# idiap/ilqr_planner

Hardware: AMD Instinct MI355X
Metric: iLQR iterations/sec (7-DoF, T=200, batch 4096) + final-cost rel-err vs Eigen ref (higher is better)
Workload: dtype f64; 1 GPU; C3: PosOrn nb_deriv=1 7-DoF Panda chain, T=200, batch 4096/GPU x 1 GPU = 4096, solver=al, 20 iterations/solve, line search on, early stop off; global_batch=4096, horizon=200, parallelism=instances sharded x1, exchange=none

## Files before the change

### ilqr_planner_amd/capi.py

```python
from __future__ import annotations

import collections
import ctypes as C
import os

import numpy as np

_HERE = os.path.dirname(os.path.abspath(__file__))
LIB_PATH = os.path.join(_HERE, "libilqr_hip.so")

MAX_SEG, MAX_KP, MAX_NX, MAX_NU, MAX_NF, MAX_NQ = 24, 8, 15, 8, 15, 13
SYS_POS_ORN, SYS_POS_ORN_TIME, SYS_JOINT, SYS_JOINT_TIME = 0, 1, 2, 3
STATUS_OK, STATUS_NONFINITE, STATUS_ALPHA_FLOOR = 0, 1, 2
LQT_MAX_NX, LQT_MAX_NU = 16, 8
CL_STATS = 5
KP_ERR, KP_STATS, CL_OUTCOME = 5, 12, 4
KP_ERR_POS, KP_ERR_ORN, KP_ERR_VEL, KP_ERR_ANGVEL, KP_ERR_TIME = range(5)
PROF_ROLLOUT, PROF_BACKWARD, PROF_FORWARD, PROF_OTHER, PROF_APPLY = 0, 1, 2, 3, 4

EXPORTS = [
    "ilqr_dims_of", "ilqr_desc_defaults", "ilqr_ctx_create", "ilqr_ctx_destroy", "ilqr_last_error", "ilqr_ctx_set_stream",
    "ilqr_ctx_synchronize", "ilqr_version", "ilqr_problem_create", "ilqr_problem_destroy", "ilqr_problem_set_init_state",
    "ilqr_problem_set_keypoint_targets", "ilqr_problem_set_controls", "ilqr_problem_set_constraints",
    "ilqr_problem_set_init_state_dev", "ilqr_problem_set_keypoint_targets_dev", "ilqr_problem_set_controls_dev",
    "ilqr_solve_recursive", "ilqr_solve_al", "ilqr_solve_batch_cp", "ilqr_solve_batch", "ilqr_problem_get_X", "ilqr_problem_get_fX",
    "ilqr_problem_get_U", "ilqr_problem_get_K", "ilqr_problem_get_d", "ilqr_problem_get_cost", "ilqr_problem_get_alpha",
    "ilqr_problem_get_iters", "ilqr_problem_get_status", "ilqr_problem_get_lambda", "ilqr_problem_get_trace",
    "ilqr_problem_get_X_dev", "ilqr_problem_get_U_dev", "ilqr_problem_get_cost_dev", "ilqr_fk_batch",
    "ilqr_profile_enable", "ilqr_profile_reset", "ilqr_profile_get", "ilqr_chain_from_urdf", "ilqr_urdf_last_error",
    "ilqr_problem_reset_multipliers", "ilqr_problem_warm_start", "ilqr_problem_track", "ilqr_problem_track_dev",
    "ilqr_problem_closed_loop", "ilqr_problem_closed_loop_dev", "ilqr_problem_closed_loop_noise", "ilqr_problem_closed_loop_noise_dev",
    "ilqr_problem_closed_loop_report", "ilqr_problem_closed_loop_report_dev",
    "ilqr_ctx_set_split", "ilqr_ctx_set_crosscheck",
    "ilqr_lqt_create", "ilqr_lqt_destroy", "ilqr_lqt_set_targets", "ilqr_lqt_set_targets_dev", "ilqr_lqt_solve_dp", "ilqr_lqt_solve_lin_al",
    "ilqr_lqt_command", "ilqr_lqt_command_dev", "ilqr_lqt_get_U", "ilqr_lqt_get_U_dev", "ilqr_lqt_get_X", "ilqr_lqt_get_X_dev", "ilqr_lqt_get_P",
    "ilqr_lqt_get_d",
]


class ProblemDesc(C.Structure):

    _fields_ = [
        ("kind", C.c_int),
        ("nb_deriv", C.c_int),
        ("dof", C.c_int),
        ("horizon", C.c_int),
        ("dt", C.c_double),
        ("R_diag", C.c_double * MAX_NU),
        ("limits_set", C.c_int),
        ("penalty", C.c_double),
        ("state_max", C.c_double * (MAX_NX + 1)),
        ("state_min", C.c_double * (MAX_NX + 1)),
        ("limit_weight", C.c_int * (MAX_NX + 1)),
        ("n_seg", C.c_int),
        ("seg_joint", C.c_int * MAX_SEG),
        ("seg_xyz", (C.c_double * 3) * MAX_SEG),
        ("seg_R", (C.c_double * 9) * MAX_SEG),
        ("seg_axis", (C.c_double * 3) * MAX_SEG),
        ("n_kp", C.c_int),
        ("kp_timestep", C.c_int * MAX_KP),
        ("kp_Q", (C.c_double * (MAX_NQ * MAX_NQ)) * MAX_KP),
        ("kp_dist", C.c_int * MAX_KP),
        ("kp_pos_radius", C.c_double * MAX_KP),
        ("kp_orn_thresh", (C.c_double * 3) * MAX_KP),
        ("kp_has_frame", C.c_int * MAX_KP),
        ("kp_frame_R", (C.c_double * 9) * MAX_KP),
# ... 33 lines not shown
class Report(C.Structure):

    _fields_ = [("kp_err", C.c_void_p), ("kp_stats", C.c_void_p), ("lim_cost", C.c_void_p), ("outcome", C.c_void_p)]


ClosedLoopNoise = collections.namedtuple("ClosedLoopNoise", "cost stats X U w")
ClosedLoopReport = collections.namedtuple("ClosedLoopReport", "cost stats kp_err kp_stats lim_cost outcome X U w")

_lib = None


def load():
    global _lib
    if _lib is not None:
        return _lib
    if not os.path.exists(LIB_PATH):
        raise RuntimeError(f"{LIB_PATH} is missing: build it with `python -c 'import __graft_entry__ as g; g.build()'` "
                           "(hipcc --offload-arch=gfx950); there is no CPU fallback")
    L = C.CDLL(LIB_PATH)
    dp, ip, vp = C.POINTER(C.c_double), C.POINTER(C.c_int), C.c_void_p
    L.ilqr_version.restype = C.c_char_p
    L.ilqr_last_error.restype = C.c_char_p
    L.ilqr_last_error.argtypes = [vp]
    L.ilqr_desc_defaults.argtypes = [C.POINTER(ProblemDesc)]
    L.ilqr_desc_defaults.restype = None
    L.ilqr_dims_of.argtypes = [C.POINTER(ProblemDesc), C.POINTER(Dims)]
    L.ilqr_ctx_create.argtypes = [C.c_int, C.POINTER(vp)]
    L.ilqr_ctx_destroy.argtypes = [vp]
    L.ilqr_ctx_destroy.restype = None
    L.ilqr_ctx_set_stream.argtypes = [vp, vp]
    L.ilqr_ctx_synchronize.argtypes = [vp]
    L.ilqr_ctx_set_split.argtypes = [vp, C.c_int]
    L.ilqr_ctx_set_crosscheck.argtypes = [vp, C.c_int, C.c_int, C.c_int, C.c_int, C.c_int, C.c_int]
    L.ilqr_problem_create.argtypes = [vp, C.POINTER(ProblemDesc), C.c_int, C.POINTER(vp)]
    L.ilqr_problem_destroy.argtypes = [vp]
    L.ilqr_problem_destroy.restype = None
    for n in ("ilqr_problem_set_init_state", "ilqr_problem_set_init_state_dev"):
        getattr(L, n).argtypes = [vp, vp, vp]
    for n in ("ilqr_problem_set_keypoint_targets", "ilqr_problem_set_keypoint_targets_dev"):
        getattr(L, n).argtypes = [vp, C.c_int, vp]
    for n in ("ilqr_problem_set_controls", "ilqr_problem_set_controls_dev"):
        getattr(L, n).argtypes = [vp, vp]
    L.ilqr_problem_set_constraints.argtypes = [vp, C.c_int, C.c_int, dp, dp, dp]
    L.ilqr_problem_reset_multipliers.argtypes = [vp]
    L.ilqr_problem_warm_start.argtypes = [vp, C.c_int]
    L.ilqr_problem_track.argtypes = [vp, C.c_int, dp, C.c_int, dp]
    L.ilqr_problem_track_dev.argtypes = [vp, C.c_int, vp, C.c_int, vp]
    L.ilqr_problem_closed_loop.argtypes = [vp, C.c_int, dp, dp, C.c_int, dp, dp, dp]
    L.ilqr_problem_closed_loop_dev.argtypes = [vp, C.c_int, vp, vp, C.c_int, vp, vp, vp]
    L.ilqr_problem_closed_loop_noise.argtypes = [vp, C.c_int, C.POINTER(Noise), dp, C.c_int, dp, dp, dp, dp, dp]
    L.ilqr_problem_closed_loop_noise_dev.argtypes = [vp, C.c_int, C.POINTER(Noise), vp, C.c_int, vp, vp, vp, vp, vp]
    L.ilqr_problem_closed_loop_report.argtypes = [vp, C.c_int, C.POINTER(Noise), dp, dp, C.c_int, C.POINTER(Tol), dp, dp, C.POINTER(Report)]
    L.ilqr_problem_closed_loop_report_dev.argtypes = [vp, C.c_int, C.POINTER(Noise), vp, vp, C.c_int, C.POINTER(Tol), vp, vp, C.POINTER(Report)]
    L.ilqr_solve_recursive.argtypes = [vp, C.c_int, C.c_int, C.c_int]
    L.ilqr_solve_al.argtypes = [vp, C.c_int, C.c_int, C.c_double, C.c_double, C.c_int, C.c_int]
    L.ilqr_solve_batch_cp.argtypes = [vp, dp, C.c_int, C.c_int, C.c_int]
    L.ilqr_solve_batch.argtypes = [vp, C.c_int, C.c_int]
    for n in ("X", "fX", "U", "K", "d", "cost", "alpha", "lambda", "X_dev", "U_dev", "cost_dev"):
        getattr(L, "ilqr_problem_get_" + n).argtypes = [vp, vp]
    L.ilqr_problem_get_iters.argtypes = [vp, ip]
    L.ilqr_problem_get_status.argtypes = [vp, ip]
    L.ilqr_problem_get_trace.argtypes = [vp, dp, dp, C.c_int]
    L.ilqr_fk_batch.argtypes = [vp, C.POINTER(ProblemDesc), C.c_int, dp, dp, dp, dp]
    L.ilqr_profile_enable.argtypes = [vp, C.c_int]
    L.ilqr_profile_reset.argtypes = [vp]
    L.ilqr_profile_get.argtypes = [vp, C.c_int, dp, ip]
# ... 103 lines not shown


class Context:
    def __init__(self, device_id: int = 0):
        import weakref

        self.L = load()
        self.h = C.c_void_p()
        self._problems = weakref.WeakSet()
        rc = self.L.ilqr_ctx_create(device_id, C.byref(self.h))
        if rc:
            raise RuntimeError(f"ilqr_ctx_create failed (code {rc}): no usable HIP device {device_id}; there is no CPU fallback")

    def check(self, rc):
        if rc:
            raise RuntimeError(self.L.ilqr_last_error(self.h).decode())

    def set_stream(self, stream_ptr):
        self.check(self.L.ilqr_ctx_set_stream(self.h, C.c_void_p(stream_ptr)))

    def synchronize(self):
        self.check(self.L.ilqr_ctx_synchronize(self.h))

    _PINS = {"sweep": {None: 0, "mfma": 1, "rows": 2}, "forward": {None: 0, "wg": 1, "dpp": 2, "wglds": 3}, "reroll": {None: 0, "rows": 1, "dpp": 2}}

    def set_crosscheck(self, generic_kernels=False, cp_lane_solve=False, cp_general=False, sweep=None, forward=None, reroll=None):
        pins = []
        for name, v in (("sweep", sweep), ("forward", forward), ("reroll", reroll)):
            if v not in self._PINS[name]:
                raise ValueError(f"set_crosscheck: {name} must be one of {[k for k in self._PINS[name] if k]} or None (got {v!r})")
            pins.append(self._PINS[name][v])
        self.check(self.L.ilqr_ctx_set_crosscheck(self.h, int(bool(generic_kernels)), int(bool(cp_lane_solve)), int(bool(cp_general)), *pins))

    def crosscheck_from_env(self):
        env = os.environ
        self.set_crosscheck(env.get("ILQR_HIP_PATH") == "v1", env.get("ILQR_CP_SOLVE") == "lane", env.get("ILQR_CP") == "general",
                            sweep=env.get("ILQR_SWEEP") or None, forward=env.get("ILQR_FWD") or None, reroll=env.get("ILQR_APPLY") or None)

    def set_split(self, mode: int):
        self.check(self.L.ilqr_ctx_set_split(self.h, int(mode)))

    def profile(self, on: bool):
        self.check(self.L.ilqr_profile_enable(self.h, int(on)))

    def profile_reset(self):
        self.check(self.L.ilqr_profile_reset(self.h))

    def profile_get(self, which):
        ms, n = C.c_double(), C.c_int()
        self.check(self.L.ilqr_profile_get(self.h, which, C.byref(ms), C.byref(n)))
        return ms.value, n.value

    def fk_batch(self, desc: ProblemDesc, q):
        q = _f64(q)
        n, dof = q.shape
        pos, quat, jac = np.zeros((n, 3)), np.zeros((n, 4)), np.zeros((n, 6, dof))
        self.check(self.L.ilqr_fk_batch(self.h, C.byref(desc), n, _dp(q), _dp(pos), _dp(quat), _dp(jac)))
        return pos, quat, jac

    def close(self):
        if self.h:
            for p in list(self._problems):
                p.close()
            self.L.ilqr_ctx_destroy(self.h)
            self.h = C.c_void_p()

    def __del__(self):
        try:
            self.close()
        except Exception:
# ... 327 lines not shown
```

### ilqr_planner_amd/csrc/ilqr_capi.cpp

```cpp
#include "../../include/ilqr_hip.h"

#include <hip/hip_runtime.h>

#include <cmath>
#include <cstdio>
#include <cstdlib>
#include <cstring>
#include <string>
#include <vector>

#include "ilqr_batchcp.hpp"
#include "ilqr_closed_loop.hpp"
#include "ilqr_ctx.hpp"
#include "ilqr_kernels.hpp"
#include "ilqr_plan.hpp"

using namespace ilqr;

struct DevScratch {
    double* ptr = nullptr;
    size_t elems = 0;
    int reserve(ilqr_ctx* c, size_t n) {
        if (elems >= n) return 0;
        if (ptr) { HIPCHK(c, hipStreamSynchronize(c->stream)); HIPCHK(c, hipFree(ptr)); ptr = nullptr; elems = 0; }
// ... 102 lines not shown
    delete c;
}

extern "C" const char* ilqr_last_error(const ilqr_ctx* c) { return c ? c->err.c_str() : "null context"; }

extern "C" int ilqr_ctx_set_stream(ilqr_ctx* c, void* s) {
    if (!c) return 1;
    c->stream = s ? (hipStream_t)s : c->own_stream;
    return 0;
}

extern "C" int ilqr_ctx_set_split(ilqr_ctx* c, int on) {
    if (!c) return 1;
    if (on < 0 || on > 2) return fail(c, "ilqr_ctx_set_split: mode must be 0, 1 or 2 (got " + std::to_string(on) + ")");
    c->split = on;
    return 0;
}

static_assert((int)SweepPin::Mfma == ILQR_XC_SWEEP_MFMA && (int)SweepPin::Rows == ILQR_XC_SWEEP_ROWS && (int)FwdPin::Wg == ILQR_XC_FWD_WG &&
              (int)FwdPin::Dpp == ILQR_XC_FWD_DPP && (int)FwdPin::WgLds == ILQR_XC_FWD_WG_LDS && (int)RerollPin::Rows == ILQR_XC_REROLL_ROWS && (int)RerollPin::Dpp == ILQR_XC_REROLL_DPP,
              "variant pins of ilqr_plan.hpp and include/ilqr_hip.h");

extern "C" int ilqr_ctx_set_crosscheck(ilqr_ctx* c, int generic_kernels, int cp_lane_solve, int cp_general, int sweep, int forward, int reroll) {
    if (!c) return 1;
    if (sweep < 0 || sweep > 2) return fail(c, "ilqr_ctx_set_crosscheck: sweep must be ILQR_XC_AUTO, ILQR_XC_SWEEP_MFMA or ILQR_XC_SWEEP_ROWS");
    if (forward < 0 || forward > 3) return fail(c, "ilqr_ctx_set_crosscheck: forward must be ILQR_XC_AUTO, ILQR_XC_FWD_WG, ILQR_XC_FWD_DPP or ILQR_XC_FWD_WG_LDS");
    if (reroll < 0 || reroll > 2) return fail(c, "ilqr_ctx_set_crosscheck: reroll must be ILQR_XC_AUTO, ILQR_XC_REROLL_ROWS or ILQR_XC_REROLL_DPP");
    c->xc_sweep = (SweepPin)sweep;
    c->xc_forward = (FwdPin)forward;
    c->xc_reroll = (RerollPin)reroll;
    c->xc_generic = generic_kernels != 0;
    c->xc_cp_lane = cp_lane_solve != 0;
    c->xc_cp_general = cp_general != 0;
    return 0;
}

extern "C" int ilqr_ctx_synchronize(ilqr_ctx* c) {
    if (!c) return 1;
    HIPCHK(c, hipStreamSynchronize(c->stream));
    return 0;
}


static hipEvent_t ev_get(ilqr_ctx* c) {
    if (!c->pool.empty()) {
        hipEvent_t e = c->pool.back();
        c->pool.pop_back();
        return e;
    }
    hipEvent_t e;
    (void)hipEventCreate(&e);
    return e;
}
static void prof_collect(ilqr_ctx* c) {
    if (c->pending.empty()) return;
    (void)hipStreamSynchronize(c->stream);
    for (size_t i = 0; i + 1 < c->pending.size(); i++) {
        const auto& p = c->pending[i];
        float ms = 0;
        if (p.which >= 0 && hipEventElapsedTime(&ms, p.a, c->pending[i + 1].a) == hipSuccess) {
            c->prof_ms[p.which] += ms;
            c->prof_n[p.which] += 1;
        }
    }
    for (auto& p : c->pending) c->pool.push_back(p.a);
    c->pending.clear();
// ... 385 lines not shown
        p->bufs.cost_trace = ct;
        p->bufs.alpha_trace = at;
        p->trace_iters = nb_iter;
    }
    if (nb_iter > 0) {
        HIPCHK(p->ctx, hipMemsetAsync(p->bufs.cost_trace, 0xFF, sizeof(double) * (size_t)nb_iter * p->Bp, p->ctx->stream));
        HIPCHK(p->ctx, hipMemsetAsync(p->bufs.alpha_trace, 0xFF, sizeof(double) * (size_t)nb_iter * p->Bp, p->ctx->stream));
    }
    return 0;
}

static Bufs half_bufs(const ilqr_problem* p, int half) {
    Bufs v = p->bufs;
    const size_t o = (size_t)p->half_b0[half];
    v.desc = p->ddesc_half[half];
    for (int i = 0; i < 2; i++) { v.X[i] += o; v.U[i] += o; }
    v.U0 += o; v.q0 += o; v.dq0 += o; v.kp_tg += o;
    v.KD += o * (size_t)kd_rs(p->bufs.kd_sym, p->dims.n_u, kd_rowp(p->dims.n_x));
    v.cost += o; v.alpha += o; v.cur += o; v.active += o; v.iters += o; v.status += o; v.kpd += o; v.pend += o; v.pred += o;
    v.lsc += o; v.dun += o; v.kpdev += o; v.kpx += o; v.dunA += o;
    if (v.ws) v.ws += o;
    if (v.cost_trace) { v.cost_trace += o; v.alpha_trace += o; }
    if (v.lambda) { v.lambda += o; v.Is += o; }
    return v;
}

static PlanIn plan_input(const ilqr_problem* p, bool al, int nb_iter, int line_search) {
    const ilqr_ctx* c = p->ctx;
    const int T = p->T;
    PlanIn in;
    in.kind = p->desc.kind; in.nd = p->desc.nb_deriv; in.al = al; in.m = p->bufs.m; in.per_step = p->bufs.per_step; in.con_state_only = p->con_state_only;
    in.limits2_set = p->desc.limits2_set != 0;
    in.shared_steps = has_shared_step(p->hdesc.steps);
    in.uniform_R = true;
    for (int i = 1; i < p->dims.n_u; i++) in.uniform_R = in.uniform_R && (p->hdesc.R_diag[i] == p->hdesc.R_diag[0]);
    in.off32 = (size_t)2 * T * p->dims.n_x * p->Bp * 8 < ((size_t)1 << 32) && (size_t)T * (p->bufs.m > 0 ? p->bufs.m : 1) * p->Bp * 8 < ((size_t)1 << 32);
    in.line_search = line_search != 0; in.alpha_floor = p->desc.alpha_floor; in.nb_iter = nb_iter;
    in.B = p->B; in.n_simd = c->n_simd; in.halves = p->ddesc_half[0] != nullptr; in.split = c->split; in.profile = c->profile;
    in.generic = c->xc_generic; in.sweep = c->xc_sweep; in.forward = c->xc_forward; in.reroll = c->xc_reroll;
    return in;
}

static int solve_riccati(ilqr_problem* p, bool al, int nb_iter, int lag, double penalty0, double scaling, int line_search, int early_stop) {
    if (!p) return 1;
    ilqr_ctx* c = p->ctx;
    if (!p->has_state || !p->has_controls) return fail(c, "set_init_state and set_controls must be called before a solve");
    if (nb_iter < 0) return fail(c, "nb_iter < 0");
    if (al && (p->bufs.m <= 0 || lag <= 0)) return fail(c, "AL solve needs constraints (ilqr_problem_set_constraints) and lag_update_step > 0");
    HIPCHK(c, hipSetDevice(c->device));
    if (ensure_trace(p, nb_iter)) return 1;
    p->last_nb_iter = nb_iter;
    p->has_gains = false;
    const int kind = p->desc.kind, nd = p->desc.nb_deriv, T = p->T;
    const RiccatiPlan pl = plan_riccati(plan_input(p, al, nb_iter, line_search));
    if (pl.kd_sym != KD_SYM_KEEP) p->bufs.kd_sym = pl.kd_sym;
    if (pl.needs_ws && !p->bufs.ws)
        if (dalloc(p, &p->bufs.ws, (size_t)backward_ws_entries(kind, nd) * p->Bp, false)) return 1;

    struct Half { Bufs bufs; int B; hipStream_t st; };
    Half hv[2];
    int nh = 1;
    if (pl.split) {
        for (int i = 0; i < 2; i++) {
            if (!c->half_stream[i]) HIPCHK(c, hipStreamCreateWithFlags(&c->half_stream[i], hipStreamNonBlocking));
            if (!c->ev_half_done[i]) HIPCHK(c, hipEventCreateWithFlags(&c->ev_half_done[i], hipEventDisableTiming));
        }
        if (!c->ev_begin) HIPCHK(c, hipEventCreateWithFlags(&c->ev_begin, hipEventDisableTiming));
        if (!c->ev_stagger) HIPCHK(c, hipEventCreateWithFlags(&c->ev_stagger, hipEventDisableTiming));
        HIPCHK(c, hipEventRecord(c->ev_begin, c->stream));
        nh = 2;
        for (int i = 0; i < 2; i++) {
            HIPCHK(c, hipStreamWaitEvent(c->half_stream[i], c->ev_begin, 0));
            hv[i].bufs = half_bufs(p, i); hv[i].B = p->half_B[i]; hv[i].st = c->half_stream[i];
        }
    } else {
        hv[0].bufs = p->bufs; hv[0].B = p->B; hv[0].st = c->stream;
    }

    struct SplitJoin {
        ilqr_ctx* c; bool on;
        ~SplitJoin() {
            if (!on) return;
            for (int i = 0; i < 2; i++)
                if (hipEventRecord(c->ev_half_done[i], c->half_stream[i]) != hipSuccess || hipStreamWaitEvent(c->stream, c->ev_half_done[i], 0) != hipSuccess)
                    (void)hipStreamSynchronize(c->half_stream[i]);
        }
    } split_join{c, pl.split};
    FwdArgs f;
    std::memset(&f, 0, sizeof(f));
    f.line_search = line_search; f.early_stop = early_stop; f.nb_iter = nb_iter; f.penalty_roll = penalty0; f.n_alpha = pl.n_alpha; f.al = al ? 1 : 0; f.n_kp = p->hdesc.steps.n;
    f.shared = has_shared_step(p->hdesc.steps) ? 1 : 0;
    f.n_kp_all = p->desc.n_kp;
    f.fused = pl.fused ? 1 : 0;
    f.fwd_lds = pl.fwd_lds ? 1 : 0;
    f.limits = p->desc.limits_set ? 1 : 0;
    for (int k = 0; k < p->desc.n_kp; k++) f.kp_ext |= p->desc.kp_dist[k] | p->desc.kp_has_frame[k] | p->desc.kp_has_Ru[k] | p->desc.kp_joint[k];
    for (int h = 0; h < nh; h++) {
        const Bufs& bf = hv[h].bufs;
        ProfScope ps(c, ILQR_PROF_ROLLOUT);
        if (pl.init == Init::Lti) launch_init_lti(kind, nd, bf, hv[h].B, hv[h].st);
        else launch_init(kind, nd, al, bf, hv[h].B, hv[h].st, penalty0);
        if (pl.init_al_update) {
            f.it = -1; f.do_update = 0;
            launch_al_update(kind, nd, bf, hv[h].B, T, hv[h].st, f);
        }
    }
    HIPCHK(c, hipGetLastError());
    double penalty = penalty0;
    SweepArgs sw;
    sw.pen_in = penalty; sw.pen_update_prev = penalty; sw.do_update_prev = 0;
    for (int it = 0; it < nb_iter; it++) {
        FwdArgs fi = f;
        fi.it = it;
        fi.penalty_roll = penalty;
        fi.do_update = al && ((it + 1) % lag == 0);
        if (fi.do_update) penalty *= scaling;
        fi.penalty_update = penalty;
        for (int h = 0; h < nh; h++) {
            const Bufs& bf = hv[h].bufs;
            const int B = hv[h].B;
            hipStream_t st = hv[h].st;
            if (pl.split && it == 0 && h == 1) HIPCHK(c, hipStreamWaitEvent(st, c->ev_stagger, 0));
            {
                ProfScope ps(c, ILQR_PROF_OTHER);
                launch_kp_derivs(kind, nd, bf, B, st, fi);
            }
            {
// ... 492 lines not shown
```

### ilqr_planner_amd/csrc/ilqr_ctx.hpp

```cpp
#pragma once
#include <hip/hip_runtime.h>

#include <string>
#include <vector>

#include "../../include/ilqr_hip.h"
#include "ilqr_plan.hpp"

struct ilqr_ctx {
    int device = 0;
    hipStream_t own_stream = nullptr;
    hipStream_t stream = nullptr;
    std::string err;
    bool profile = false;
    int split = 1;
    double prof_ms[ILQR_PROF_COUNT] = {0, 0, 0, 0, 0};
    int prof_n[ILQR_PROF_COUNT] = {0, 0, 0, 0, 0};
    struct Pending { hipEvent_t a, b; int which; };
    std::vector<Pending> pending;
    std::vector<hipEvent_t> pool;
    std::vector<ilqr_problem*> problems;
    struct Cleanup { void (*destroy)(void*); void* handle; };
    std::vector<Cleanup> cleanups;
    int n_simd = 1024;
    bool xc_generic = false, xc_cp_lane = false, xc_cp_general = false;
    ilqr::SweepPin xc_sweep = ilqr::SweepPin::Auto;
    ilqr::FwdPin xc_forward = ilqr::FwdPin::Auto;
    ilqr::RerollPin xc_reroll = ilqr::RerollPin::Auto;
    hipStream_t half_stream[2] = {nullptr, nullptr};
    hipEvent_t ev_begin = nullptr, ev_half_done[2] = {nullptr, nullptr}, ev_stagger = nullptr;
};

static inline int fail(ilqr_ctx* c, const std::string& m) {
    if (c) c->err = m;
    return 1;
}
#define HIPCHK(ctx, call)                                                                                  \
    do {                                                                                                   \
        hipError_t e_ = (call);                                                                            \
        if (e_ != hipSuccess) return fail((ctx), std::string(#call) + ": " + hipGetErrorString(e_));       \
    } while (0)
```

### ilqr_planner_amd/csrc/ilqr_kernels.hip

```cpp
#include "ilqr_closed_loop.hpp"
#include "ilqr_kernels.hpp"
#include "ilqr_step.hpp"

namespace ilqr {


#define NOUNR _Pragma("unroll 1")

template <class S, bool AL>
__global__ __launch_bounds__(64) void k_init_rollout(Bufs a, double penalty) {
    constexpr int NX = S::NX, NU = S::NU;
    const DevDesc& d = *a.desc;
    const int b = blockIdx.x * 64 + threadIdx.x;
    if (b >= d.B) return;
    const int Bp = d.Bp, T = d.T;
    double x[NX], u[NU], xn[NX];
    init_state<S>(d, a, b, x);
    double cost = 0;
    int st = 0;
    double* X = a.X[0];
    double* U = a.U[0];
    for (int k = 0; k < T - 1; k++) {
        UNR for (int i = 0; i < NX; i++) AT(X, k * NX + i, b) = x[i];
        UNR for (int i = 0; i < NU; i++) { u[i] = AT(a.U0, k * NU + i, b); AT(U, k * NU + i, b) = u[i]; }
        if (AL) {
            for (int r = 0; r < a.m; r++) {
                double g = con_g<S>(a, k, r, x, u);
                double lam = AT(a.lambda, k * a.m + r, b);
                AT(a.Is, k * a.m + r, b) = penalty * ((g < 0 && lam == 0) ? 0.0 : 1.0);
            }
        }
        const bool iskp = (st < d.steps.n && d.steps.t[st] == k);
        cost += stage_cost<S>(d, a, b, iskp ? st : -1, x, u);
        if (iskp) st++;
// ... 758 lines not shown
template <class S>
__global__ __launch_bounds__(64) void k_fx_all(Bufs a, double* __restrict__ out ) {
    const DevDesc& d = *a.desc;
    const int b = blockIdx.x * blockDim.x + threadIdx.x;
    const int t = blockIdx.y;
    if (b >= d.B) return;
    const int Bp = d.Bp;
    const double* X = a.X[a.cur[b]];
    double x[S::NX], fxv[S::NF];
    UNR for (int i = 0; i < S::NX; i++) x[i] = AT(X, t * S::NX + i, b);
    fx_of<S, false>(d, x, fxv, nullptr);
    UNR for (int i = 0; i < S::NF; i++) out[((size_t)b * d.T + t) * S::NF + i] = fxv[i];
}

__global__ __launch_bounds__(64) void k_fk_batch(const DevDesc* dd, int n, const double* __restrict__ q, double* __restrict__ pos, double* __restrict__ quat,
                           double* __restrict__ jac) {
    const int i = blockIdx.x * blockDim.x + threadIdx.x;
    if (i >= n) return;
    double qv[DOF], p[3], qt[4], J[6][DOF];
    UNR for (int j = 0; j < DOF; j++) qv[j] = q[(size_t)i * DOF + j];
    fk<true>(dd->chain, qv, p, qt, J);
    if (pos) { UNR for (int j = 0; j < 3; j++) pos[(size_t)i * 3 + j] = p[j]; }
    if (quat) { UNR for (int j = 0; j < 4; j++) quat[(size_t)i * 4 + j] = qt[j]; }
    if (jac) {
        UNR for (int r = 0; r < 6; r++)
            UNR for (int j = 0; j < DOF; j++) jac[((size_t)i * 6 + r) * DOF + j] = J[r][j];
    }
}



void launch_kp_derivs(int kind, int nd, const Bufs& a, int B, hipStream_t st, const FwdArgs& f) {
    if (f.n_kp <= 0) return;
    SysAll::dispatch(kind, nd, [&](auto s) {
        using S = decltype(s);
        if (f.shared) {
            hipLaunchKernelGGL((k_kp_terms<S>), dim3((B + 63) / 64, f.n_kp_all), dim3(64), 0, st, a);
            hipLaunchKernelGGL((k_kp_sum<S>), dim3((B + 63) / 64, f.n_kp), dim3(64), 0, st, a);
        } else if (f.kp_ext) hipLaunchKernelGGL((k_kp_derivs<S, true>), dim3((B + 63) / 64, f.n_kp), dim3(64), 0, st, a, f.fused);
        else hipLaunchKernelGGL((k_kp_derivs<S, false>), dim3((B + 63) / 64, f.n_kp), dim3(64), 0, st, a, f.fused);
    });
}

void launch_init(int kind, int nd, bool al, const Bufs& a, int B, hipStream_t st, double penalty) {
    SysAll::dispatch(kind, nd, [&](auto s) {
        using S = decltype(s);
        if (al) hipLaunchKernelGGL((k_init_rollout<S, true>), dim3((B + 63) / 64), dim3(64), 0, st, a, penalty);
        else hipLaunchKernelGGL((k_init_rollout<S, false>), dim3((B + 63) / 64), dim3(64), 0, st, a, penalty);
    });
}

void launch_backward_generic(int kind, int nd, bool al, const Bufs& a, int B, hipStream_t st) {
    SysAll::dispatch(kind, nd, [&](auto s) {
        using S = decltype(s);
        if (al) hipLaunchKernelGGL((k_backward<S, true>), dim3((B + 63) / 64), dim3(64), 0, st, a);
        else hipLaunchKernelGGL((k_backward<S, false>), dim3((B + 63) / 64), dim3(64), 0, st, a);
    });
}

void launch_forward_generic(int kind, int nd, bool al, const Bufs& a, int B, hipStream_t st, const FwdArgs& f) {
    SysAll::dispatch(kind, nd, [&](auto s) {
        using S = decltype(s);
        if (al)
            hipLaunchKernelGGL((k_forward<S, true>), dim3((B + 63) / 64), dim3(64), 0, st, a, f.it, f.line_search, f.early_stop, f.penalty_roll,
                               f.penalty_update, f.do_update, f.nb_iter);
        else
// ... 76 lines not shown
```

### ilqr_planner_amd/csrc/ilqr_kernels.hpp

```cpp
#pragma once
#include <hip/hip_runtime.h>

#include "ilqr_device.hpp"
#include "ilqr_dofmap.hpp"

namespace ilqr {

struct Bufs {
    const DevDesc* desc;
    double* X[2];
    double* U[2];
    const double* U0;
    double* KD;
    const double* q0;
    const double* dq0;
    const double* kp_tg;
    double* cost;
    double* alpha;
    int* cur;
    int* active;
    int* iters;
    int* status;
    double* kpd;
    int* pend;
// ... 3 lines not shown
    double* kpdev;
    double* kpx;
    double* dunA;
    double* ws;
    double* cost_trace;
    double* alpha_trace;
    int m, per_step;
    const double* conA;
    const double* conb;
    double* lambda;
    double* Is;
    int kd_sym;
};

constexpr int kd_rowp(int nx) { return (nx + 2) & ~1; }
constexpr int KD_SYM_RS = 36, KD_SYM_D = 28;
__host__ __device__ constexpr int kd_sym_tri(int i, int j) { return i * 7 - i * (i - 1) / 2 + (j - i); }
__host__ __device__ constexpr int kd_sym_off(int i, int j) { return j >= 7 ? KD_SYM_D + i : (i <= j ? kd_sym_tri(i, j) : kd_sym_tri(j, i)); }
__host__ __device__ inline int kd_off(int sym, int rowp, int i, int j) { return sym ? kd_sym_off(i, j) : i * rowp + j; }
__host__ __device__ inline int kd_rs(int sym, int nu, int rowp) { return sym ? KD_SYM_RS : nu * rowp; }
#define KD_REC(kd, Bp, RS, k, b) ((kd) + ((size_t)(k) * (size_t)(Bp) + (size_t)(b)) * (size_t)(RS))

struct FwdArgs {
    int it, line_search, early_stop, do_update, nb_iter;
    int n_kp;
    int shared;
    int n_kp_all;
    int al;
    int n_alpha;
    double penalty_roll, penalty_update;
    int kp_ext;
    int limits;
    int fused;
    int fwd_lds;
};

struct SweepArgs {
    double pen_in;
    double pen_update_prev;
    int do_update_prev;
};

void launch_init(int kind, int nd, bool al, const Bufs& a, int B, hipStream_t st, double penalty);
void launch_kp_derivs(int kind, int nd, const Bufs& a, int B, hipStream_t st, const FwdArgs& f);
void launch_backward_generic(int kind, int nd, bool al, const Bufs& a, int B, hipStream_t st);
int backward_ws_entries(int kind, int nd);
void launch_forward_generic(int kind, int nd, bool al, const Bufs& a, int B, hipStream_t st, const FwdArgs& f);
void launch_init_lti(int kind, int nd, const Bufs& a, int B, hipStream_t st);
void launch_backward_si_dpp(bool al, bool fused, bool uniform_R, int lpi, const Bufs& a, int B, hipStream_t st, const SweepArgs& sw);
void launch_backward_rows(int kind, int nd, bool al, const Bufs& a, int B, hipStream_t st);
void launch_backward_mfma(int kind, int nd, bool al, const Bufs& a, int B, hipStream_t st);
void launch_forward_wave(int kind, bool small, const Bufs& a, int B, hipStream_t st, const FwdArgs& f);
void launch_apply_wave(int kind, const Bufs& a, int B, int T, hipStream_t st, const FwdArgs& f);
void launch_forward_lin(const Bufs& a, int B, hipStream_t st, const FwdArgs& f);
void launch_apply_lin(const Bufs& a, int B, int T, hipStream_t st);
void launch_forward_tm(int kind, int nd, const Bufs& a, int B, hipStream_t st, const FwdArgs& f);
void launch_apply_tm(int kind, int nd, bool dpp, const Bufs& a, int B, hipStream_t st, const FwdArgs& f);
void launch_al_update(int kind, int nd, const Bufs& a, int B, int T, hipStream_t st, const FwdArgs& f);
void launch_fx_all(int kind, int nd, const Bufs& a, int B, int T, double* out, hipStream_t st);
void launch_to_soa(const double* src, double* dst, int B, int Bp, int rows, hipStream_t st);
void launch_from_soa(const double* src, double* dst, int B, int Bp, int rows, hipStream_t st);
void launch_from_soa_cur(const double* s0, const double* s1, const int* cur, double* dst, int B, int Bp, int rows, hipStream_t st);
void launch_from_soa_scaled(const double* src, const double* alpha, const int* iters, double* dst, int B, int Bp, int rows, hipStream_t st);
void launch_get_gains(const double* kd, int kd_sym, const double* alpha, const int* iters, double* K_out, double* d_out, int B, int Bp, int T1, int nu, int nx, hipStream_t st);
void launch_warm_start(const Bufs& a, double* U0, double* q0, double* dq0, int shift, int B, int T, int nx, int nu, int nd, hipStream_t st);
void launch_track(const Bufs& a, const double* x_meas, int k, int with_ff, double* u_out, int B, int nx, int nu, hipStream_t st);
void launch_closed_loop_stats(const double* cost, int B, int S, double* stats, hipStream_t st);
void launch_fk_batch(const DevDesc* dd, int n, const double* q, double* pos, double* quat, double* jac, hipStream_t st);
void launch_to_soa_map(const double* src, double* dst, int B, int Bp, int outer, const IndexMap& m, hipStream_t st);
void launch_from_soa_cur_map(const double* s0, const double* s1, const int* cur, double* dst, int B, int Bp, int outer, const IndexMap& m,
                             hipStream_t st);
void launch_get_gains_map(const double* kd, int kd_sym, const double* alpha, const int* iters, double* K_out, double* d_out, int B, int Bp, int T1,
                          const DofMap& m, hipStream_t st);
void launch_track_map(const Bufs& a, const double* x_meas, int k, int with_ff, double* u_out, int B, const DofMap& m, hipStream_t st);

}
```

### ilqr_planner_amd/csrc/ilqr_plan.hpp

```cpp
#pragma once

namespace ilqr {

constexpr int SPLIT_MIN_BATCH = 2048;
constexpr int split_first_half(int B) { return (B / 2 + 63) / 64 * 64; }


constexpr bool backward_si_supported(int kind, int nd, bool al, int m, int per_step, bool con_state_only) {
    return (kind == 0 || kind == 2) && nd == 1 && (!al || (con_state_only && per_step == 0 && m <= 4));
}
constexpr bool backward_mfma_supported(int kind, int , bool al, int m) { return kind != 2 && (!al || m <= 16); }
constexpr bool backward_rows_supported(int kind, int nd, bool al, int m) {
    return kind != 2 && !(kind == 0 && nd == 1) && (!al || m <= 16);
}
constexpr bool forward_wave_supported(int kind, int nd, int n_alpha) { return (kind == 0 || kind == 2) && nd == 1 && n_alpha <= 16; }
constexpr bool forward_lin_supported(int kind, int nd, int n_alpha) { return kind == 0 && nd == 2 && n_alpha <= 16; }
constexpr bool init_lti_supported(int kind, int nd) {
    return ((kind == 0 || kind == 1) && (nd == 1 || nd == 2)) || ((kind == 2 || kind == 3) && nd == 1);
}

inline int n_alpha_of(bool line_search, double alpha_floor) {
    int n = 1;
    if (line_search) { double a = 1.0; while (a > alpha_floor && n < 64) { a *= 0.5; n++; } }
    return n;
}

constexpr int si_lanes(int launched_B, int n_simd) { return (launched_B + 3) / 4 <= n_simd ? 16 : 8; }

enum class SweepPin { Auto = 0, Mfma = 1, Rows = 2 };
enum class FwdPin { Auto = 0, Wg = 1, Dpp = 2, WgLds = 3 };
enum class RerollPin { Auto = 0, Rows = 1, Dpp = 2 };

struct PlanIn {
    int kind = 0, nd = 1;
    bool al = false;
    int m = 0, per_step = 0;
    bool con_state_only = false;
    bool limits2_set = false;
    bool shared_steps = false;
    bool uniform_R = false;
    bool off32 = true;
    bool line_search = true;
    double alpha_floor = 1e-3;
    int nb_iter = 0;
    int B = 0, n_simd = 1024;
    bool halves = false;
    int split = 1;
    bool profile = false;
    bool generic = false;
    SweepPin sweep = SweepPin::Auto;
    FwdPin forward = FwdPin::Auto;
    RerollPin reroll = RerollPin::Auto;
};

enum class Init { Lti, Generic };
enum class Sweep { SiDpp, Mfma, Rows, Generic };
enum class Forward { WaveWg, WaveDpp, Lin, Mfma, Generic };
enum class Apply {
    None,
    Wave,
    WaveLast,
    Lin,
    RerollRows,
    RerollDpp,
};
constexpr int KD_SYM_KEEP = -1;

struct RiccatiPlan {
    int n_alpha = 1;
    Init init = Init::Generic;
    bool init_al_update = false;
    Sweep sweep = Sweep::Generic;
    int si_lanes[2] = {16, 16};
    Forward forward = Forward::Generic;
    bool fwd_lds = false;
    Apply apply = Apply::None;
    bool al_update = false;
    bool fused = false;
    int kd_sym = 0;
    bool split = false;
    bool needs_ws = false;
};

inline RiccatiPlan plan_riccati(const PlanIn& in) {
    RiccatiPlan p;
    const int kind = in.kind, nd = in.nd;
    p.n_alpha = n_alpha_of(in.line_search, in.alpha_floor);
    const bool cooperative = !in.generic && !in.limits2_set && !in.shared_steps;
    const bool coop_fwd = cooperative && p.n_alpha <= 16;

    if (cooperative && in.off32 && backward_si_supported(kind, nd, in.al, in.m, in.per_step, in.con_state_only)) p.sweep = Sweep::SiDpp;
    else if (cooperative && backward_mfma_supported(kind, nd, in.al, in.m)) {
        const bool rows = in.sweep == SweepPin::Rows || (in.sweep == SweepPin::Auto && in.B > 2 * in.n_simd);
        p.sweep = rows && backward_rows_supported(kind, nd, in.al, in.m) ? Sweep::Rows : Sweep::Mfma;
    }

    if (coop_fwd && forward_wave_supported(kind, nd, p.n_alpha)) {
        const bool dpp = in.forward == FwdPin::Dpp || (in.forward == FwdPin::Auto && (in.B + 3) / 4 <= 3 * in.n_simd / 4);
        p.forward = dpp ? Forward::WaveDpp : Forward::WaveWg;
        p.fwd_lds = in.forward == FwdPin::WgLds;
    } else if (coop_fwd && forward_lin_supported(kind, nd, p.n_alpha)) {
        p.forward = Forward::Lin;
    } else if (coop_fwd) {
        p.forward = Forward::Mfma;
    }
    const bool wave = p.forward == Forward::WaveWg || p.forward == Forward::WaveDpp;
    p.fused = p.sweep == Sweep::SiDpp && wave;
    p.kd_sym = in.nb_iter == 0 ? KD_SYM_KEEP : (p.fused && in.uniform_R) ? 1 : 0;

    if (wave) p.apply = p.fused ? Apply::WaveLast : Apply::Wave;
    else if (p.forward == Forward::Lin) p.apply = Apply::Lin;
    else if (p.forward == Forward::Mfma && in.line_search) {
        const bool dpp = in.reroll == RerollPin::Dpp || (in.reroll == RerollPin::Auto && (in.B + 3) / 4 <= in.n_simd / 4);
        p.apply = dpp ? Apply::RerollDpp : Apply::RerollRows;
    }
    p.al_update = in.al && coop_fwd && !wave;

    p.init = cooperative && init_lti_supported(kind, nd) ? Init::Lti : Init::Generic;
    p.init_al_update = p.init == Init::Lti && in.al && !p.fused;

    p.split = coop_fwd && ((p.sweep == Sweep::Mfma && in.split) || in.split == 2) && !in.profile && in.halves && in.nb_iter > 0;
    p.needs_ws = p.sweep == Sweep::Generic && in.nb_iter > 0;
    const int b0 = p.split ? split_first_half(in.B) : in.B;
    p.si_lanes[0] = si_lanes(b0, in.n_simd);
    p.si_lanes[1] = si_lanes(in.B - b0, in.n_simd);
    return p;
}

}
```

### include/ilqr_hip.h

```cpp
#ifndef ILQR_HIP_H
#define ILQR_HIP_H

#include <stddef.h>

#ifdef __cplusplus
extern "C" {
#endif

#define ILQR_MAX_SEG 24
#define ILQR_MAX_KP 8
#define ILQR_MAX_NX 15
#define ILQR_MAX_NU 8
#define ILQR_MAX_NF 15
#define ILQR_MAX_NQ 13

#define ILQR_SYS_POS_ORN 0
#define ILQR_SYS_POS_ORN_TIME 1
#define ILQR_SYS_JOINT 2
#define ILQR_SYS_JOINT_TIME 3

#define ILQR_STATUS_OK 0
#define ILQR_STATUS_NONFINITE 1
#define ILQR_STATUS_ALPHA_FLOOR 2

// ... 34 lines not shown
    double penalty2;
    double state_max2[ILQR_MAX_NX + 1];
    double state_min2[ILQR_MAX_NX + 1];
    int limit_weight2[ILQR_MAX_NX + 1];
    int limit_multiplicity2;
    double reg;
    double alpha_floor;
    double stop_tol;
} ilqr_problem_desc;

typedef struct { int n_x, n_u, n_f, n_Q; } ilqr_dims;
int ilqr_dims_of(const ilqr_problem_desc* desc, ilqr_dims* out);
void ilqr_desc_defaults(ilqr_problem_desc* desc);

int ilqr_chain_from_urdf(const char* urdf_text, const char* base_frame, const char* tip_frame, const double* tool_rpy,
                         const double* tool_xyz, ilqr_problem_desc* desc, double* lower, double* upper);
const char* ilqr_urdf_last_error(void);

int ilqr_ctx_create(int device_id, ilqr_ctx** out);
void ilqr_ctx_destroy(ilqr_ctx* ctx);
const char* ilqr_last_error(const ilqr_ctx* ctx);
int ilqr_ctx_set_stream(ilqr_ctx* ctx, void* hip_stream);
int ilqr_ctx_synchronize(ilqr_ctx* ctx);
int ilqr_ctx_set_split(ilqr_ctx* ctx, int on);
#define ILQR_XC_AUTO 0
#define ILQR_XC_SWEEP_MFMA 1
#define ILQR_XC_SWEEP_ROWS 2
#define ILQR_XC_FWD_WG 1
#define ILQR_XC_FWD_DPP 2
#define ILQR_XC_FWD_WG_LDS 3
#define ILQR_XC_REROLL_ROWS 1
#define ILQR_XC_REROLL_DPP 2
int ilqr_ctx_set_crosscheck(ilqr_ctx* ctx, int generic_kernels, int cp_lane_solve, int cp_general, int sweep, int forward, int reroll);
const char* ilqr_version(void);

int ilqr_problem_create(ilqr_ctx* ctx, const ilqr_problem_desc* desc, int batch, ilqr_problem** out);
void ilqr_problem_destroy(ilqr_problem* p);

int ilqr_problem_set_init_state(ilqr_problem* p, const double* q0, const double* dq0);
int ilqr_problem_set_keypoint_targets(ilqr_problem* p, int kp_index, const double* target);
int ilqr_problem_set_controls(ilqr_problem* p, const double* U0);
int ilqr_problem_set_constraints(ilqr_problem* p, int m, int per_step, const double* A, const double* b, const double* lambda0);
int ilqr_problem_reset_multipliers(ilqr_problem* p);
int ilqr_problem_set_init_state_dev(ilqr_problem* p, const double* q0, const double* dq0);
int ilqr_problem_set_keypoint_targets_dev(ilqr_problem* p, int kp_index, const double* target);
int ilqr_problem_set_controls_dev(ilqr_problem* p, const double* U0);

int ilqr_solve_recursive(ilqr_problem* p, int nb_iter, int line_search, int early_stop);
int ilqr_solve_al(ilqr_problem* p, int nb_iter, int lag_update_step, double penalty, double scaling_factor,
                  int line_search, int early_stop);
int ilqr_solve_batch_cp(ilqr_problem* p, const double* psi, int Kw, int nb_iter, int early_stop);
int ilqr_solve_batch(ilqr_problem* p, int nb_iter, int early_stop);

int ilqr_problem_get_X(ilqr_problem* p, double* X);
int ilqr_problem_get_fX(ilqr_problem* p, double* fX);
int ilqr_problem_get_U(ilqr_problem* p, double* U);
int ilqr_problem_get_K(ilqr_problem* p, double* K);
int ilqr_problem_get_d(ilqr_problem* p, double* d);
int ilqr_problem_get_cost(ilqr_problem* p, double* cost);
int ilqr_problem_get_alpha(ilqr_problem* p, double* alpha);
int ilqr_problem_get_iters(ilqr_problem* p, int* iters);
int ilqr_problem_get_status(ilqr_problem* p, int* status);
int ilqr_problem_get_lambda(ilqr_problem* p, double* lambda);
int ilqr_problem_get_trace(ilqr_problem* p, double* cost_trace, double* alpha_trace, int nb_iter);
int ilqr_problem_get_X_dev(ilqr_problem* p, double* X);
int ilqr_problem_get_U_dev(ilqr_problem* p, double* U);
// ... 78 lines not shown
```

Before: 13.07 million problem-iterations/s.

## Add lane-parallel keypoint-derivative kernel for first-order PosOrn chains

Adds a keypoint-derivative kernel that assigns eight lanes to each instance. Each lane computes its own joint's rotation, shares it through LDS, and builds its own Jacobian column and one row of the Gauss-Newton Hessian. The plan picks it automatically for first-order PosOrn problems with no extended keypoint features when the batch is small relative to the SIMD count. The aim is more parallelism and shorter per-instance latency than the one-lane-per-instance path. In exchange, every lane redundantly walks the full forward kinematics chain, and the change adds an environment/API pin to select the variant.

```diff
diff --git a/ilqr_planner_amd/capi.py b/ilqr_planner_amd/capi.py
--- a/ilqr_planner_amd/capi.py
+++ b/ilqr_planner_amd/capi.py
@@ -31,7 +31,7 @@
     "ilqr_problem_reset_multipliers", "ilqr_problem_warm_start", "ilqr_problem_track", "ilqr_problem_track_dev",
     "ilqr_problem_closed_loop", "ilqr_problem_closed_loop_dev", "ilqr_problem_closed_loop_noise", "ilqr_problem_closed_loop_noise_dev",
     "ilqr_problem_closed_loop_report", "ilqr_problem_closed_loop_report_dev",
-    "ilqr_ctx_set_split", "ilqr_ctx_set_crosscheck",
+    "ilqr_ctx_set_split", "ilqr_ctx_set_crosscheck", "ilqr_ctx_set_kp_derivs",
     "ilqr_lqt_create", "ilqr_lqt_destroy", "ilqr_lqt_set_targets", "ilqr_lqt_set_targets_dev", "ilqr_lqt_solve_dp", "ilqr_lqt_solve_lin_al",
     "ilqr_lqt_command", "ilqr_lqt_command_dev", "ilqr_lqt_get_U", "ilqr_lqt_get_U_dev", "ilqr_lqt_get_X", "ilqr_lqt_get_X_dev", "ilqr_lqt_get_P",
     "ilqr_lqt_get_d",
@@ -131,6 +131,7 @@
     L.ilqr_ctx_synchronize.argtypes = [vp]
     L.ilqr_ctx_set_split.argtypes = [vp, C.c_int]
     L.ilqr_ctx_set_crosscheck.argtypes = [vp, C.c_int, C.c_int, C.c_int, C.c_int, C.c_int, C.c_int]
+    L.ilqr_ctx_set_kp_derivs.argtypes = [vp, C.c_int]
     L.ilqr_problem_create.argtypes = [vp, C.POINTER(ProblemDesc), C.c_int, C.POINTER(vp)]
     L.ilqr_problem_destroy.argtypes = [vp]
     L.ilqr_problem_destroy.restype = None
@@ -300,10 +301,18 @@
             pins.append(self._PINS[name][v])
         self.check(self.L.ilqr_ctx_set_crosscheck(self.h, int(bool(generic_kernels)), int(bool(cp_lane_solve)), int(bool(cp_general)), *pins))
 
+    _KPD = {None: 0, "lanes": 1, "lane": 2}
+
+    def set_kp_derivs(self, variant=None):
+        if variant not in self._KPD:
+            raise ValueError(f"set_kp_derivs: variant must be 'lanes', 'lane' or None (got {variant!r})")
+        self.check(self.L.ilqr_ctx_set_kp_derivs(self.h, self._KPD[variant]))
+
     def crosscheck_from_env(self):
         env = os.environ
         self.set_crosscheck(env.get("ILQR_HIP_PATH") == "v1", env.get("ILQR_CP_SOLVE") == "lane", env.get("ILQR_CP") == "general",
                             sweep=env.get("ILQR_SWEEP") or None, forward=env.get("ILQR_FWD") or None, reroll=env.get("ILQR_APPLY") or None)
+        self.set_kp_derivs(env.get("ILQR_KPD") or None)
 
     def set_split(self, mode: int):
         self.check(self.L.ilqr_ctx_set_split(self.h, int(mode)))
diff --git a/ilqr_planner_amd/csrc/ilqr_capi.cpp b/ilqr_planner_amd/csrc/ilqr_capi.cpp
--- a/ilqr_planner_amd/csrc/ilqr_capi.cpp
+++ b/ilqr_planner_amd/csrc/ilqr_capi.cpp
@@ -158,6 +158,15 @@
     c->xc_generic = generic_kernels != 0;
     c->xc_cp_lane = cp_lane_solve != 0;
     c->xc_cp_general = cp_general != 0;
+    return 0;
+}
+
+static_assert((int)KpdPin::Auto == ILQR_KPD_AUTO && (int)KpdPin::Lanes == ILQR_KPD_LANES && (int)KpdPin::Lane == ILQR_KPD_LANE, "ilqr_plan.hpp and include/ilqr_hip.h");
+
+extern "C" int ilqr_ctx_set_kp_derivs(ilqr_ctx* c, int variant) {
+    if (!c) return 1;
+    if (variant < 0 || variant > 2) return fail(c, "ilqr_ctx_set_kp_derivs: variant must be ILQR_KPD_AUTO, ILQR_KPD_LANES or ILQR_KPD_LANE (got " + std::to_string(variant) + ")");
+    c->xc_kpd = (KpdPin)variant;
     return 0;
 }
 
@@ -609,12 +618,13 @@
     in.kind = p->desc.kind; in.nd = p->desc.nb_deriv; in.al = al; in.m = p->bufs.m; in.per_step = p->bufs.per_step; in.con_state_only = p->con_state_only;
     in.limits2_set = p->desc.limits2_set != 0;
     in.shared_steps = has_shared_step(p->hdesc.steps);
+    for (int k = 0; k < p->desc.n_kp; k++) in.kp_ext = in.kp_ext || p->desc.kp_dist[k] || p->desc.kp_has_frame[k] || p->desc.kp_has_Ru[k] || p->desc.kp_joint[k];
     in.uniform_R = true;
     for (int i = 1; i < p->dims.n_u; i++) in.uniform_R = in.uniform_R && (p->hdesc.R_diag[i] == p->hdesc.R_diag[0]);
     in.off32 = (size_t)2 * T * p->dims.n_x * p->Bp * 8 < ((size_t)1 << 32) && (size_t)T * (p->bufs.m > 0 ? p->bufs.m : 1) * p->Bp * 8 < ((size_t)1 << 32);
     in.line_search = line_search != 0; in.alpha_floor = p->desc.alpha_floor; in.nb_iter = nb_iter;
     in.B = p->B; in.n_simd = c->n_simd; in.halves = p->ddesc_half[0] != nullptr; in.split = c->split; in.profile = c->profile;
-    in.generic = c->xc_generic; in.sweep = c->xc_sweep; in.forward = c->xc_forward; in.reroll = c->xc_reroll;
+    in.generic = c->xc_generic; in.sweep = c->xc_sweep; in.forward = c->xc_forward; in.reroll = c->xc_reroll; in.kpd = c->xc_kpd;
     return in;
 }
 
@@ -670,6 +680,7 @@
     f.n_kp_all = p->desc.n_kp;
     f.fused = pl.fused ? 1 : 0;
     f.fwd_lds = pl.fwd_lds ? 1 : 0;
+    f.kp_lanes = pl.kp_lanes ? 1 : 0;
     f.limits = p->desc.limits_set ? 1 : 0;
     for (int k = 0; k < p->desc.n_kp; k++) f.kp_ext |= p->desc.kp_dist[k] | p->desc.kp_has_frame[k] | p->desc.kp_has_Ru[k] | p->desc.kp_joint[k];
     for (int h = 0; h < nh; h++) {
diff --git a/ilqr_planner_amd/csrc/ilqr_ctx.hpp b/ilqr_planner_amd/csrc/ilqr_ctx.hpp
--- a/ilqr_planner_amd/csrc/ilqr_ctx.hpp
+++ b/ilqr_planner_amd/csrc/ilqr_ctx.hpp
@@ -27,6 +27,7 @@
     ilqr::SweepPin xc_sweep = ilqr::SweepPin::Auto;
     ilqr::FwdPin xc_forward = ilqr::FwdPin::Auto;
     ilqr::RerollPin xc_reroll = ilqr::RerollPin::Auto;
+    ilqr::KpdPin xc_kpd = ilqr::KpdPin::Auto;
     hipStream_t half_stream[2] = {nullptr, nullptr};
     hipEvent_t ev_begin = nullptr, ev_half_done[2] = {nullptr, nullptr}, ev_stagger = nullptr;
 };
diff --git a/ilqr_planner_amd/csrc/ilqr_kernels.hip b/ilqr_planner_amd/csrc/ilqr_kernels.hip
--- a/ilqr_planner_amd/csrc/ilqr_kernels.hip
+++ b/ilqr_planner_amd/csrc/ilqr_kernels.hip
@@ -1,5 +1,6 @@
 #include "ilqr_closed_loop.hpp"
 #include "ilqr_kernels.hpp"
+#include "ilqr_plan.hpp"
 #include "ilqr_step.hpp"
 
 namespace ilqr {
@@ -824,6 +825,9 @@
 
 void launch_kp_derivs(int kind, int nd, const Bufs& a, int B, hipStream_t st, const FwdArgs& f) {
     if (f.n_kp <= 0) return;
+#if defined(__HIPCC__)
+    if (f.kp_lanes && !f.shared && !f.kp_ext && kp_lanes_supported(kind, nd)) { launch_kp_derivs_lanes(a, B, st, f); return; }
+#endif
     SysAll::dispatch(kind, nd, [&](auto s) {
         using S = decltype(s);
         if (f.shared) {
diff --git a/ilqr_planner_amd/csrc/ilqr_kernels.hpp b/ilqr_planner_amd/csrc/ilqr_kernels.hpp
--- a/ilqr_planner_amd/csrc/ilqr_kernels.hpp
+++ b/ilqr_planner_amd/csrc/ilqr_kernels.hpp
@@ -59,6 +59,7 @@
     int kp_ext;
     int limits;
     int fused;
+    int kp_lanes;
     int fwd_lds;
 };
 
@@ -73,6 +74,7 @@
 void launch_backward_generic(int kind, int nd, bool al, const Bufs& a, int B, hipStream_t st);
 int backward_ws_entries(int kind, int nd);
 void launch_forward_generic(int kind, int nd, bool al, const Bufs& a, int B, hipStream_t st, const FwdArgs& f);
+void launch_kp_derivs_lanes(const Bufs& a, int B, hipStream_t st, const FwdArgs& f);
 void launch_init_lti(int kind, int nd, const Bufs& a, int B, hipStream_t st);
 void launch_backward_si_dpp(bool al, bool fused, bool uniform_R, int lpi, const Bufs& a, int B, hipStream_t st, const SweepArgs& sw);
 void launch_backward_rows(int kind, int nd, bool al, const Bufs& a, int B, hipStream_t st);
diff --git a/ilqr_planner_amd/csrc/ilqr_kernels_kplanes.hip b/ilqr_planner_amd/csrc/ilqr_kernels_kplanes.hip
--- /dev/null
+++ b/ilqr_planner_amd/csrc/ilqr_kernels_kplanes.hip
@@ -0,0 +1,151 @@
+#include "ilqr_kernels.hpp"
+#include "ilqr_lanes.hpp"
+#include "ilqr_step.hpp"
+
+namespace ilqr {
+
+using KS = Sys<0, 1>;
+constexpr int KPL_RQ = 9 * DOF;
+constexpr int KPL_GROUP = KPL_RQ + 6 * DOF;
+
+__global__ __launch_bounds__(64) void k_kp_derivs_lanes(Bufs a, int fused) {
+    using S = KS;
+    constexpr int NX = S::NX, NF = S::NF, NQ = S::NQ;
+    static_assert(NX == DOF && NQ == 6 && NF == 7, "first-order PosOrn only");
+    __shared__ double sh[8][KPL_GROUP];
+    const DevDesc& d = *a.desc;
+    const int g = threadIdx.x >> 3, me = threadIdx.x & 7;
+    const int jj = me < DOF ? me : DOF - 1;
+    const int b = xcd_tile() * 8 + g;
+    const int kpi = blockIdx.y;
+    if (b >= d.B) return;
+    if (!a.active[b]) return;
+    const int Bp = d.Bp;
+    const int k = d.kp_t[kpi];
+    const int cur = a.cur[b];
+    const double* X = a.X[cur];
+    const double* X1 = a.X[1 - cur];
+    const int w = fused ? a.pend[b] - 1 : -1;
+    auto state = [&](int i) {
+        double xi = AT(X, k * NX + i, b);
+        if (w >= 0) {
+            const double aa = ldexp(1.0, -w);
+            const double x1 = AT(X1, k * NX + i, b);
+            xi = (w == 0) ? x1 : fma(aa, x1 - xi, xi);
+        }
+        return xi;
+    };
+    const double xme = state(jj);
+    auto finish = [&](double* row, double lxi) {
+        if (d.limits_set && d.lw[jj] != 0) {
+            double qv = 0, L = 0;
+            if (xme > d.smax[jj]) { qv = d.smax[jj] - xme; L = d.penalty; }
+            else if (xme < d.smin[jj]) { qv = d.smin[jj] - xme; L = d.penalty; }
+            lxi += -L * qv;
+            UNR for (int j = 0; j < NX; j++) {
+                const double v = row[j] + ((L != 0.0) ? d.pen_xx : 0.0);
+                row[j] = (j == jj) ? v : row[j];
+            }
+        }
+        if (me < DOF) {
+            double* out = a.kpd + (size_t)kpi * (NX + NX * NX) * Bp;
+            AT(out, me, b) = lxi;
+            UNR for (int j = 0; j < NX; j++) AT(out, NX + me * NX + j, b) = row[j];
+        }
+    };
+    const DevChain& c = d.chain;
+    double* sRq = sh[g];
+    double* sJ = sh[g] + KPL_RQ;
+
+    {
+        const double x = c.axis[jj][0], y = c.axis[jj][1], z = c.axis[jj][2];
+        double st, ct;
+        sincos(xme, &st, &ct);
+        double vt = 1 - ct;
+        double Rq[9] = {ct + vt * x * x,      -z * st + vt * x * y, y * st + vt * x * z,
+                        z * st + vt * x * y,  ct + vt * y * y,      -x * st + vt * y * z,
+                        -y * st + vt * x * z, x * st + vt * y * z,  ct + vt * z * z};
+        if (me < DOF) {
+            UNR for (int i = 0; i < 9; i++) sRq[9 * me + i] = Rq[i];
+        }
+    }
+    LDS_ORDER();
+
+    double R[9] = {1, 0, 0, 0, 1, 0, 0, 0, 1}, pos[3] = {0, 0, 0};
+    double org[3] = {0, 0, 0}, ax[3] = {0, 0, 0};
+    double Rqn[9];
+    UNR for (int i = 0; i < 9; i++) Rqn[i] = sRq[i];
+#pragma unroll 1
+    for (int j = 0; j < DOF; j++) {
+        double Rq[9], Rn[9];
+        UNR for (int i = 0; i < 9; i++) Rq[i] = Rqn[i];
+        const int jn = j + 1 < DOF ? j + 1 : j;
+        UNR for (int i = 0; i < 9; i++) Rqn[i] = sRq[9 * jn + i];
+        UNR for (int i = 0; i < 3; i++) pos[i] += R[3 * i] * c.ppre[j][0] + R[3 * i + 1] * c.ppre[j][1] + R[3 * i + 2] * c.ppre[j][2];
+        mat3_mul(R, c.Rpre[j], Rn);
+        const double x = c.axis[j][0], y = c.axis[j][1], z = c.axis[j][2];
+        UNR for (int i = 0; i < 3; i++) {
+            const double axi = Rn[3 * i] * x + Rn[3 * i + 1] * y + Rn[3 * i + 2] * z;
+            org[i] = (j == jj) ? pos[i] : org[i];
+            ax[i] = (j == jj) ? axi : ax[i];
+        }
+        mat3_mul(Rn, Rq, R);
+    }
+    double fxv[NF];
+    {
+        double Rn[9];
+        UNR for (int i = 0; i < 3; i++) pos[i] += R[3 * i] * c.ptail[0] + R[3 * i + 1] * c.ptail[1] + R[3 * i + 2] * c.ptail[2];
+        mat3_mul(R, c.Rtail, Rn);
+        kdl_quat(Rn, fxv + 3);
+    }
+    fxv[0] = pos[0]; fxv[1] = pos[1]; fxv[2] = pos[2];
+
+    double Jc[6];
+    {
+        double r0 = pos[0] - org[0], r1 = pos[1] - org[1], r2 = pos[2] - org[2];
+        Jc[0] = ax[1] * r2 - ax[2] * r1;
+        Jc[1] = ax[2] * r0 - ax[0] * r2;
+        Jc[2] = ax[0] * r1 - ax[1] * r0;
+        Jc[3] = ax[0];
+        Jc[4] = ax[1];
+        Jc[5] = ax[2];
+    }
+    if (me < DOF) {
+        UNR for (int r = 0; r < 6; r++) sJ[r * DOF + me] = Jc[r];
+    }
+    LDS_ORDER();
+    double J[6][DOF];
+    UNR for (int r = 0; r < 6; r++)
+        UNR for (int j = 0; j < DOF; j++) J[r][j] = sJ[r * DOF + j];
+
+    double e[NQ], tg[NF], Qe[NQ];
+    UNR for (int i = 0; i < NF; i++) tg[i] = AT(a.kp_tg, kpi * NF + i, b);
+    kp_diff<S>(tg, fxv, e);
+    const double* Q = d.kp_Q[kpi];
+    UNR for (int i = 0; i < NQ; i++) {
+        double s = 0;
+        UNR for (int j = 0; j < NQ; j++) s += Q[i * NQ + j] * e[j];
+        Qe[i] = s;
+    }
+    double sl = 0;
+    UNR for (int r = 0; r < 6; r++) sl += Jc[r] * Qe[r];
+    double jq[NQ], row[NX];
+    UNR for (int rp = 0; rp < NQ; rp++) {
+        double s = 0;
+        UNR for (int r = 0; r < 6; r++) s += Jc[r] * Q[r * NQ + rp];
+        jq[rp] = s;
+    }
+    UNR for (int c2 = 0; c2 < DOF; c2++) {
+        double s = 0;
+        UNR for (int r = 0; r < 6; r++) s += jq[r] * J[r][c2];
+        row[c2] = 0.0 + s;
+    }
+    finish(row, 0.0 + -1 * sl);
+}
+
+void launch_kp_derivs_lanes(const Bufs& a, int B, hipStream_t st, const FwdArgs& f) {
+    const dim3 grid(grid_x8((unsigned)(B + 7) / 8u), f.n_kp);
+    hipLaunchKernelGGL(k_kp_derivs_lanes, grid, dim3(64), 0, st, a, f.fused);
+}
+
+}
diff --git a/ilqr_planner_amd/csrc/ilqr_plan.hpp b/ilqr_planner_amd/csrc/ilqr_plan.hpp
--- a/ilqr_planner_amd/csrc/ilqr_plan.hpp
+++ b/ilqr_planner_amd/csrc/ilqr_plan.hpp
@@ -27,6 +27,13 @@
 
 constexpr int si_lanes(int launched_B, int n_simd) { return (launched_B + 3) / 4 <= n_simd ? 16 : 8; }
 
+constexpr bool kp_lanes_supported(int kind, int nd) { return kind == 0 && nd == 1; }
+enum class KpdPin { Auto = 0, Lanes = 1, Lane = 2 };
+constexpr int KP_LANES_MAX_PER_SIMD = 8;
+constexpr bool kp_lanes_of(int kind, int nd, int B, int n_simd, KpdPin pin) {
+    return kp_lanes_supported(kind, nd) && pin != KpdPin::Lane && (pin == KpdPin::Lanes || B <= KP_LANES_MAX_PER_SIMD * n_simd);
+}
+
 enum class SweepPin { Auto = 0, Mfma = 1, Rows = 2 };
 enum class FwdPin { Auto = 0, Wg = 1, Dpp = 2, WgLds = 3 };
 enum class RerollPin { Auto = 0, Rows = 1, Dpp = 2 };
@@ -37,6 +44,7 @@
     int m = 0, per_step = 0;
     bool con_state_only = false;
     bool limits2_set = false;
+    bool kp_ext = false;
     bool shared_steps = false;
     bool uniform_R = false;
     bool off32 = true;
@@ -51,6 +59,7 @@
     SweepPin sweep = SweepPin::Auto;
     FwdPin forward = FwdPin::Auto;
     RerollPin reroll = RerollPin::Auto;
+    KpdPin kpd = KpdPin::Auto;
 };
 
 enum class Init { Lti, Generic };
@@ -79,6 +88,7 @@
     bool fused = false;
     int kd_sym = 0;
     bool split = false;
+    bool kp_lanes = false;
     bool needs_ws = false;
 };
 
@@ -121,6 +131,7 @@
 
     p.split = coop_fwd && ((p.sweep == Sweep::Mfma && in.split) || in.split == 2) && !in.profile && in.halves && in.nb_iter > 0;
     p.needs_ws = p.sweep == Sweep::Generic && in.nb_iter > 0;
+    p.kp_lanes = !in.generic && !in.shared_steps && !in.kp_ext && kp_lanes_of(kind, nd, in.B, in.n_simd, in.kpd);
     const int b0 = p.split ? split_first_half(in.B) : in.B;
     p.si_lanes[0] = si_lanes(b0, in.n_simd);
     p.si_lanes[1] = si_lanes(in.B - b0, in.n_simd);
diff --git a/include/ilqr_hip.h b/include/ilqr_hip.h
--- a/include/ilqr_hip.h
+++ b/include/ilqr_hip.h
@@ -90,6 +90,10 @@
 #define ILQR_XC_REROLL_ROWS 1
 #define ILQR_XC_REROLL_DPP 2
 int ilqr_ctx_set_crosscheck(ilqr_ctx* ctx, int generic_kernels, int cp_lane_solve, int cp_general, int sweep, int forward, int reroll);
+#define ILQR_KPD_AUTO 0
+#define ILQR_KPD_LANES 1
+#define ILQR_KPD_LANE 2
+int ilqr_ctx_set_kp_derivs(ilqr_ctx* ctx, int variant);
 const char* ilqr_version(void);
 
 int ilqr_problem_create(ilqr_ctx* ctx, const ilqr_problem_desc* desc, int batch, ilqr_problem** out);
```

Result: no change. 13.18 million problem-iterations/s, median of 6 (+0.9%).
